# Francis-Fan-create/SCaSML_GP

Measured on AMD Instinct MI355X. Metric: Euler-Maruyama path-steps/sec + L2 rel-error, Grad_Dependent_Nonlinear d=100 n=3, higher is better.
Workload: dtype f32

## Files before the change

### scasml_gp_amd/csrc/gp_eval_compat_mfma.hip

```cpp
#include <stdlib.h>
#include <type_traits>

#include "gp_common.hpp"
#include "gp_mfma16.hpp"

namespace scasml {

constexpr int kHutch = 5;

typedef _Float16 h16x2 __attribute__((ext_vector_type(2)));
typedef float f32x2 __attribute__((ext_vector_type(2)));

struct CompatIdxF {
    int32_t i[kHutch];
};

struct GpCompatArgs {
    const float *points;
    const float *model;
    int32_t idx[kHutch];
    float4 *out4;
    float *lap;
    int64_t n_inf;
    int32_t n_pad, kp, d, first_bdy_tile;
    float a, sigma, mu;
    int32_t eq_id;
    int32_t round_out;
    const uint8_t *site_kinds;
    int64_t rows_per_site;
    const int32_t *site_order;
    int32_t n_listed;
};

template <bool R16>
struct Pair {
    using T = std::conditional_t<R16, h16x2, f32x2>;
    T v;
    __device__ __forceinline__ Pair(float a, float b) {
        if constexpr (R16) v = __builtin_convertvector((f32x2){a, b}, h16x2);
        else v = (f32x2){a, b};
    }
    __device__ __forceinline__ float lo() const { return (float)v.x; }
    __device__ __forceinline__ float hi() const { return (float)v.y; }
};

__device__ __forceinline__ float pin(float x) {
    asm("" : "+v"(x));
    return x;
}

template <int KS, int PLANES>
__device__ __forceinline__ void compat_mfma_lam(const float4 *lds_a, const s16x8 (&xb)[PLANES][KS], f32x16 &acc, int lane, float acc0) {
#pragma unroll
    for (int r = 0; r < 16; ++r) acc[r] = acc0;
    constexpr int NA = PLANES == 2 ? 1 : 2;
    Frag a[NA];
    if constexpr (NA == 2) a[0].f = lds_a[lane];
#pragma unroll
    for (int s = 0; s < KS; ++s) {
        const int cur = NA == 2 ? (s & 1) : 0, nxt = cur ^ 1;
        if constexpr (NA == 2) {
            if (s + 1 < KS) a[nxt].f = lds_a[(s + 1) * 64 + lane];
        } else {
            a[0].f = lds_a[s * 64 + lane];
        }
        Frag b0;
        b0.v = xb[0][s];
        if constexpr (PLANES == 2) {
            Frag b1;
            b1.v = xb[1][s];
            acc = __builtin_amdgcn_mfma_f32_32x32x16_f16(a[cur].h, b1.h, acc, 0, 0, 0);
        }
        acc = __builtin_amdgcn_mfma_f32_32x32x16_f16(a[cur].h, b0.h, acc, 0, 0, 0);
        __builtin_amdgcn_sched_barrier(0);
    }
}

struct CompatPoint {
    float sx, tx, ax0, sx2, wxa, wxb;
};
struct CompatConsts {
    float a, ad, c4, c10;
};

template <int GEOM, int FORM, bool BDY, bool R16>
__device__ __forceinline__ void compat_epilogue(const float *rows_lds, const f32x16 &lam, const f32x16 &G, int half, const CompatPoint &p,
                                                const CompatConsts &c, float &au, float &at, float &ad, float &al) {
    const float4 *cb = reinterpret_cast<const float4 *>(__builtin_assume_aligned(rows_lds + 4 * 8 * half, 16));
    constexpr int NQ = (BDY || GEOM == 1) ? 1 : 2;
    float4 q[1][NQ];
    auto fetch = [&](int r, float4 (&dst)[NQ]) {
        const int row = (r & 3) + 8 * (r >> 2);
#pragma unroll
        for (int i = 0; i < NQ; ++i) dst[i] = cb[row * 2 + i];
    };
#pragma unroll
    for (int r = 0; r < 16; ++r) {
        const int cur = 0;
        fetch(r, q[0]);
        __builtin_amdgcn_sched_barrier(0);
        const float kap = pin(__builtin_amdgcn_exp2f(lam[r]));
        if constexpr (GEOM == 0) {
            const float vsy = q[cur][0].x, vty = q[cur][0].y, c0 = q[cur][0].z;
            if constexpr (BDY && FORM == 1) {
                const Pair<R16> k0(kap, 0.0f);
                au = fmaf(c0, k0.lo(), au);
            } else {
                const float pp = p.tx - vty, ss = p.sx - vsy;
                const float e1 = pin(pp * kap), e2 = pin(ss * kap);
                if constexpr (BDY) {
                    const Pair<R16> k01(kap, e1), k2(e2, 0.0f);
                    au = fmaf(c0, k01.lo(), au);
                    if constexpr (FORM == 0) at = fmaf(-c0, k01.hi(), at);
                    if constexpr (FORM != 1) ad = fmaf(-c0, k2.lo(), ad);
                } else {
                    const float cL = q[cur][0].w, ct = q[cur][1].x, cS = q[cur][1].y;
                    if constexpr (FORM == 1) {
                        const Pair<R16> k01(kap, e1), k2(e2, 0.0f);
                        au = fmaf(cS, k2.lo(), fmaf(ct, k01.hi(), fmaf(c0, k01.lo(), au)));
                    } else {
                        const float e4 = pin(pp * e2);
                        const float e5 = pin(fmaf(-ss, e2, c.ad * kap));
                        if constexpr (FORM == 2) {
                            const Pair<R16> k01(kap, e1), k24(e2, e4), k5(e5, 0.0f);
                            au = fmaf(cS, k24.lo(), fmaf(ct, k01.hi(), fmaf(c0, k01.lo(), au)));
                            ad = fmaf(cS, k5.lo(), fmaf(-ct, k24.hi(), fmaf(-c0, k24.lo(), ad)));
                        } else {
                            const float e3 = fmaf(-pp, e1, c.a * kap);
                            const float g0 = G[r];
                            const float e6 = fmaf(g0, g0 - c.c4, -c.c10) * kap;
                            const Pair<R16> k01(kap, e1), k23(e2, e3), k45(e4, e5), k6(e6, 0.0f);
                            au = fmaf(cS, k23.lo(), fmaf(ct, k01.hi(), fmaf(c0, k01.lo(), au)));
                            at = fmaf(-cS, k45.lo(), fmaf(ct, k23.hi(), fmaf(-c0, k01.hi(), at)));
                            ad = fmaf(cS, k45.hi(), fmaf(-ct, k45.lo(), fmaf(-c0, k23.lo(), ad)));
                            al = fmaf(cL, k6.lo(), al);
                        }
                    }
                }
            }
        } else if constexpr (GEOM == 1) {
            const float vsy1 = q[cur][0].x, vay0 = q[cur][0].y, vwy1 = q[cur][0].z, cL = q[cur][0].w;
            const float g1 = G[r];
            const float f1 = pin(g1 * kap);
            if constexpr (FORM == 1) {
                const Pair<R16> k1(f1, 0.0f);
                au = fmaf(cL, k1.lo(), au);
            } else {
                const float m = fmaf(-(p.sx - vsy1), g1, p.wxb - vwy1);
                const float f3 = pin(m * kap);
                if constexpr (FORM == 2) {
                    const Pair<R16> k13(f1, f3);
                    au = fmaf(cL, k13.lo(), au);
                    ad = fmaf(cL, k13.hi(), ad);
                } else {
                    const float f2 = (p.tx - vay0) * f1;
                    const Pair<R16> k12(f1, f2), k3(f3, 0.0f);
                    au = fmaf(cL, k12.lo(), au);
                    at = fmaf(-cL, k12.hi(), at);
                    ad = fmaf(cL, k3.lo(), ad);
                }
            }
        } else {
            const float vsy = q[cur][0].x, vty = q[cur][0].y, vwy2 = q[cur][0].z, c0 = q[cur][0].w;
            const float g2 = G[r];
            const float h1 = g2 * kap;
            if constexpr (BDY) {
                const Pair<R16> k1(h1, 0.0f);
                al = fmaf(c0, k1.lo(), al);
            } else {
                const float ct = q[cur][1].x, cS = q[cur][1].y;
                const float h2 = (p.ax0 - vty) * h1;
                const float m = fmaf(-(p.sx2 - vsy), g2, p.wxa - vwy2);
                const float h3 = m * kap;
                const Pair<R16> k12(h1, h2), k3(h3, 0.0f);
                al = fmaf(-cS, k3.lo(), fmaf(ct, k12.hi(), fmaf(c0, k12.lo(), al)));
            }
        }
    }
}

template <int GEOM, int FORM, bool BDY>
__device__ __forceinline__ void compat_epilogue_fact(const float *rows_lds, const f32x16 &lam, const f32x16 &G, int half, const CompatPoint &p,
                                                     const CompatConsts &c, float &au, float &at, float &ad, float &al) {
    const float4 *cb = reinterpret_cast<const float4 *>(__builtin_assume_aligned(rows_lds + 4 * 8 * half, 16));
    constexpr int Q0 = GEOM == 2 ? 1 : 0;
    constexpr int NQ = (GEOM == 0 && !BDY) ? 2 : 1;
    float4 q[2][NQ];
    auto fetch = [&](int r, float4 (&dst)[NQ]) {
        const int row = (r & 3) + 8 * (r >> 2);
#pragma unroll
        for (int i = 0; i < NQ; ++i) dst[i] = cb[row * 2 + Q0 + i];
    };
    fetch(0, q[0]);
#pragma unroll
    for (int r = 0; r < 16; ++r) {
        const int cur = r & 1, nxt = cur ^ 1;
        if (r + 1 < 16) fetch(r + 1, q[nxt]);
        #ifndef SCASML_FACT_NOSCHED
        __builtin_amdgcn_sched_barrier(0);
#endif
        const float kap = __builtin_amdgcn_exp2f(lam[r]);
        if constexpr (GEOM == 0) {
            const float vsy = q[cur][0].x, vty = q[cur][0].y, c0 = q[cur][0].z;
            if constexpr (BDY) {
                const float F = c0 * kap;
                au += F;
                if constexpr (FORM == 0) at = fmaf(-(p.tx - vty), F, at);
                if constexpr (FORM != 1) ad = fmaf(-(p.sx - vsy), F, ad);
            } else {
                const float cL = q[cur][0].w, ct = q[cur][1].x, cS = q[cur][1].y;
                const float pp = p.tx - vty, ss = p.sx - vsy;
                const float E = fmaf(ct, pp, fmaf(cS, ss, c0));
                au = fmaf(kap, E, au);
                if constexpr (FORM != 1) ad = fmaf(kap, fmaf(-ss, E, q[cur][1].w), ad);
                if constexpr (FORM == 0) {
                    at = fmaf(kap, fmaf(-pp, E, q[cur][1].z), at);
                    const float g0 = G[r];
                    al = fmaf(cL * kap, fmaf(g0, g0 - c.c4, -c.c10), al);
                }
            }
        } else if constexpr (GEOM == 1) {
            const float vsy1 = q[cur][0].x, vay0 = q[cur][0].y, vwy1 = q[cur][0].z, cL = q[cur][0].w;
            const float v = cL * kap;
            if constexpr (FORM == 1) {
                au = fmaf(v, G[r], au);
            } else {
                const float w = v * G[r];
                au += w;
                ad = fmaf(-(p.sx - vsy1), w, fmaf(v, p.wxb - vwy1, ad));
                if constexpr (FORM == 0) at = fmaf(-(p.tx - vay0), w, at);
            }
        } else {
            const float ct = q[cur][0].x, cS = q[cur][0].y, e0 = q[cur][0].z, cSw = q[cur][0].w;
            if constexpr (BDY) {
                al = fmaf(kap * G[r], e0, al);
            } else {
                const float E2 = fmaf(ct, p.ax0, fmaf(cS, p.sx2, e0));
                const float t = fmaf(cS, p.wxa, -cSw);
                al = fmaf(kap, fmaf(G[r], E2, -t), al);
            }
        }
    }
}

constexpr int kStageTail = 256 + 256;

template <int KS, int BPC, bool R16, int PLANES>
__global__ __launch_bounds__(256, BPC) void gp_eval_compat_mfma_kernel(const GpCompatArgs g) {
    static_assert(PLANES == 2 || !R16, "the as-coded form keeps both point planes");
#ifndef SCASML_COMPAT_NSLOT
#define SCASML_COMPAT_NSLOT 3
#endif
    constexpr int WPB = 4, NSLOT = SCASML_COMPAT_NSLOT, AHEAD = 2;
    constexpr int STAGE = KS * 256 + kStageTail;
    constexpr int NCHUNK = STAGE / 256;
    constexpr int CLO = NCHUNK / WPB, CREM = NCHUNK % WPB;
    extern __shared__ __attribute__((aligned(16))) float lds[];
    const int lane = threadIdx.x & 63, wv = threadIdx.x >> 6;
    const int col = lane & 31, half = lane >> 5;
    const int64_t blk = blockIdx.x;
    int64_t p0 = (blk * WPB + wv) * 32;
    const int n_tiles = g.n_pad / 32;
    const int nb0 = g.first_bdy_tile < n_tiles ? g.first_bdy_tile : n_tiles;

    int form_listed = -1;
    if (g.site_order) {
        const int64_t wps = g.rows_per_site >> 5;
        bool all_u = true, all_ud = true;
        for (int w = 0; w < WPB; ++w) {
            const int64_t vs = (blk * WPB + w) / wps;
            if (vs >= g.n_listed) continue;
            const int k = g.site_kinds ? g.site_kinds[g.site_order[vs]] : 0;
            if (!(k == 1 || k == 3)) all_u = false;
            if (!(k == 1 || k == 3 || k == 4)) all_ud = false;
        }
        form_listed = all_u ? 1 : (all_ud ? 2 : 0);
        const int64_t vw = blk * WPB + wv, vs = vw / wps;
        p0 = vs < g.n_listed ? (int64_t)g.site_order[vs] * g.rows_per_site + (vw - vs * wps) * 32 : g.n_inf;
    }

    if (!g.site_order && g.site_kinds && g.rows_per_site >= 32) {
        const int64_t b0 = blk * WPB * 32;
        if (b0 < g.n_inf) {
            const int64_t b1 = (b0 + WPB * 32 < g.n_inf ? b0 + WPB * 32 : g.n_inf) - 1;
            bool unowned = true;
            for (int64_t s = b0 / g.rows_per_site; s <= b1 / g.rows_per_site; ++s)
                if (g.site_kinds[s] != 2) unowned = false;
            if (unowned) return;
        }
    }
    int form = 0;
    if (g.site_order) {
        form = form_listed;
    } else if (g.site_kinds && g.rows_per_site >= 32) {
        const int64_t b0 = blk * WPB * 32;
        const int64_t b1 = (b0 + WPB * 32 < g.n_inf ? b0 + WPB * 32 : g.n_inf) - 1;
        if (b0 < g.n_inf) {
            bool all_u = true, all_ud = true;
            for (int64_t s = b0 / g.rows_per_site; s <= b1 / g.rows_per_site; ++s) {
                const int k = g.site_kinds[s];
                if (k == 2) continue;
                if (!(k == 1 || k == 3)) all_u = false;
                if (!(k == 1 || k == 3 || k == 4)) all_ud = false;
            }
            form = all_u ? 1 : (all_ud ? 2 : 0);
        }
    }
    form = __builtin_amdgcn_readfirstlane(form);
    const int GD = form == 0 ? 3 : 2, GB = form == 0 ? 2 : 1;
    const int n_stages = nb0 * GD + (n_tiles - nb0) * GB;

    const int wvs = __builtin_amdgcn_readfirstlane(wv);
    const bool extra = wvs < CREM;
    const uint32_t lds_base = __builtin_amdgcn_readfirstlane((uint32_t)(uintptr_t)lds);
    auto stage_src = [&](int s) -> const float * {
        int tile, geom;
        if (s < nb0 * GD) {
            tile = s / GD;
            geom = s - tile * GD;
        } else {
            const int t = s - nb0 * GD;
            tile = nb0 + t / GB;
            geom = form == 0 ? 2 * (t - (t / GB) * GB) : 0;
        }
        return g.model + ((int64_t)tile * 3 + geom) * STAGE;
    };
    auto stage = [&](int s) {
        const uint32_t dst = lds_base + (uint32_t)((s % NSLOT) * STAGE) * 4u;
        const float *src = stage_src(s);
        auto chunk = [&](int c) { glds16_asm(src + c * 256, (uint32_t)lane * 16u, dst + (uint32_t)c * 1024u); };
#pragma unroll
        for (int i = 0; i < CLO; ++i) chunk(wvs + i * WPB);
        if (CREM && extra) chunk(wvs + CLO * WPB);
    };
    auto rendezvous = [&](bool newest_may_fly) {
        if (newest_may_fly) {
            if (CREM && extra) {
                asm volatile("s_waitcnt vmcnt(%0)" ::"n"(CLO + 1) : "memory");
            } else {
                asm volatile("s_waitcnt vmcnt(%0)" ::"n"(CLO) : "memory");
            }
        } else {
            asm volatile("s_waitcnt vmcnt(0)" ::: "memory");
        }
        __builtin_amdgcn_s_barrier();
        asm volatile("" ::: "memory");
    };
    stage(0);
    if (n_stages > 1) stage(1);

    const float qs = 0.5f * 1.44269504088896341f / g.a, k1 = -qs;
    const float hh = (float)g.d / (float)kHutch;
    const float ha2 = hh * g.a * g.a;
    s16x8 xb[PLANES][KS];
    float acc0 = 0.0f;
    CompatPoint pt;
    Frag qa[1], qb[1];
    {
        int64_t row = p0 + col;
        if (row >= g.n_inf) row = g.n_inf - 1;
        const float *prow = g.points + row * g.kp;
        const int kbase = half * (8 * KS);
        const float4 *src = reinterpret_cast<const float4 *>(prow + kbase);
        float pn = 0.0f, ps = 0.0f;
        const float ptime = prow[g.d], px0 = prow[0];
        const float fold = 2.0f * g.a * g.a * qs;
        auto make_planes = [&](const float (&t)[8], Frag &fh, Frag &fl) {
#pragma unroll
            for (int c = 0; c < 4; ++c) {
                const float h0 = (float)(_Float16)t[2 * c], h1 = (float)(_Float16)t[2 * c + 1];
                fh.u[c] = pack_h2(t[2 * c], t[2 * c + 1]);
                fl.u[c] = pack_h2(t[2 * c] - h0, t[2 * c + 1] - h1);
            }
        };
        float tlast[8];
#pragma unroll
        for (int s = 0; s < KS; ++s) {
            const float4 q0 = src[2 * s], q1 = src[2 * s + 1];
            const float e[8] = {q0.x, q0.y, q0.z, q0.w, q1.x, q1.y, q1.z, q1.w};
            float t[8];
#pragma unroll
            for (int c2 = 0; c2 < 8; ++c2) {
                pn = fmaf(e[c2], e[c2], pn);
                ps += e[c2];
                t[c2] = fold * e[c2];
            }
            if (s == KS - 1) {
#pragma unroll
                for (int c2 = 0; c2 < 8; ++c2) tlast[c2] = t[c2];
            } else {
                Frag fh, fl;
                make_planes(t, fh, fl);
                xb[0][s] = fh.v;
                if constexpr (PLANES == 2) xb[1][s] = fl.v;
            }
        }
        pn += __shfl_xor(pn, 32);
        ps += __shfl_xor(ps, 32);
        tlast[5] = half ? 1.0f : tlast[5];
        tlast[6] = half ? 1.0f : tlast[6];
        tlast[7] = half ? k1 * g.a * g.a * pn : tlast[7];
        {
            Frag fh, fl;
            make_planes(tlast, fh, fl);
            xb[0][KS - 1] = fh.v;
            if constexpr (PLANES == 2) xb[1][KS - 1] = fl.v;
            else acc0 = k1 * g.a * g.a * pn - (float)(_Float16)(k1 * g.a * g.a * pn);
        }
        pt.sx = g.a * (ps - ptime);
        pt.tx = g.a * ptime;
        pt.ax0 = g.a * px0;
        pt.sx2 = pt.sx - pt.ax0 + pt.tx;
        float ua[kHutch], ub[kHutch], sa = 0.0f, sb = 0.0f, na = 0.0f, nb = 0.0f;
#pragma unroll
        for (int j = 0; j < kHutch; ++j) {
            const float va = prow[g.idx[j] + 1], vb = prow[g.idx[j]];
            sa += va;
            sb += vb;
            na = fmaf(va, va, na);
            nb = fmaf(vb, vb, nb);
            ua[j] = -2.0f * ha2 * va;
            ub[j] = -2.0f * ha2 * vb;
        }
        pt.wxa = 2.0f * ha2 * sa;
        pt.wxb = 2.0f * ha2 * sb;
        auto qfrag = [&](const float (&u)[kHutch], float px, Frag &f) {
            auto hi = [](float v) { return (float)(_Float16)v; };
            if (half == 0) {
                f.u[0] = pack_h2(u[0], u[1]);
                f.u[1] = pack_h2(u[2], u[3]);
                f.u[2] = pack_h2(u[4], px);
                f.u[3] = pack_h2(px - hi(px), 1.0f);
            } else {
                f.u[0] = pack_h2(u[0] - hi(u[0]), u[1] - hi(u[1]));
                f.u[1] = pack_h2(u[2] - hi(u[2]), u[3] - hi(u[3]));
                f.u[2] = pack_h2(u[4] - hi(u[4]), 1.0f);
                f.u[3] = 0u;
            }
        };
        const float c5ah = (float)kHutch * g.a * hh;
        qfrag(ua, fmaf(ha2, na, -c5ah), qa[0]);
        qfrag(ub, fmaf(ha2, nb, -c5ah), qb[0]);
    }
    CompatConsts cc;
    cc.a = g.a;
    cc.ad = g.a * (float)g.d;
    cc.c4 = 4.0f * g.a * hh;
    cc.c10 = 10.0f * g.a * g.a * hh * hh;
    float au = 0.0f, at = 0.0f, ad = 0.0f, al = 0.0f;
    f32x16 acc, accG;
    uint32_t region;
    asm volatile("s_mov_b32 %0, -1" : "=s"(region));

    int s_now = 0;
    auto step = [&](auto geom_c, auto form_c, auto bdy_c) {
        constexpr int GEOM = decltype(geom_c)::value, FORM = decltype(form_c)::value;
        constexpr bool BDY = decltype(bdy_c)::value;
        constexpr bool NEEDG = GEOM != 0 || (FORM == 0 && !BDY);
        const int slot = s_now % NSLOT;
        if (s_now + AHEAD < n_stages) stage(s_now + AHEAD);
        const float *base = lds + slot * STAGE;
        if (region & 1) {
            compat_mfma_lam<KS, PLANES>(reinterpret_cast<const float4 *>(base), xb, acc, lane, acc0);
            if constexpr (NEEDG) {
                Frag aq;
                aq.f = reinterpret_cast<const float4 *>(base + KS * 256)[lane];
#pragma unroll
                for (int r = 0; r < 16; ++r) accG[r] = 0.0f;
                accG = __builtin_amdgcn_mfma_f32_32x32x16_f16(aq.h, GEOM == 1 ? qb[0].h : qa[0].h, accG, 0, 0, 0);
            }
        }
        if (region & 2) {
            if constexpr (R16) compat_epilogue<GEOM, FORM, BDY, true>(base + (KS + 1) * 256, acc, accG, half, pt, cc, au, at, ad, al);
            else compat_epilogue_fact<GEOM, FORM, BDY>(base + (KS + 1) * 256, acc, accG, half, pt, cc, au, at, ad, al);
        }
        rendezvous(s_now + AHEAD < n_stages);
        ++s_now;
    };
    using I0 = std::integral_constant<int, 0>;
    using I1 = std::integral_constant<int, 1>;
    using I2 = std::integral_constant<int, 2>;
    auto sweep = [&](auto form_c) {
        constexpr int FORM = decltype(form_c)::value;
        for (int jt = 0; jt < nb0; ++jt) {
            step(I0{}, form_c, std::false_type{});
            step(I1{}, form_c, std::false_type{});
            if constexpr (FORM == 0) step(I2{}, form_c, std::false_type{});
        }
        for (int jt = nb0; jt < n_tiles; ++jt) {
            step(I0{}, form_c, std::true_type{});
            if constexpr (FORM == 0) step(I2{}, form_c, std::true_type{});
        }
    };
    rendezvous(n_stages > 1);
    if (form == 2) sweep(I2{});
    else if (form == 1) sweep(I1{});
    else sweep(I0{});

    float u = au + __shfl_xor(au, 32);
    const float dt = at + __shfl_xor(at, 32);
    const float dv = ad + __shfl_xor(ad, 32);
    const float lp = al + __shfl_xor(al, 32);
    const int64_t row = p0 + col;
    if (half == 0 && row < g.n_inf) {
        if (g.round_out) u = (float)(_Float16)u;
        float eps = dt + g.mu * dv + 0.5f * g.sigma * g.sigma * lp + eq_f<float>(g.eq_id, u, g.sigma * dv, g.sigma, (float)g.d);
        if (g.round_out) eps = (float)(_Float16)eps;
        g.out4[row] = make_float4(u, dv, eps, dt);
        if (g.lap) g.lap[row] = lp;
    }
}

__global__ void gp_compat_pack_mfma_kernel(int d, float a, const float *x_dom, int n_dom, const float *x_bdy, int n_bdy, const double *rv,
                                           CompatIdxF ix, float *model, int n_pad, int kp) {
    const int j = blockIdx.x * blockDim.x + threadIdx.x;
    if (j >= n_pad) return;
    const int N = n_dom + n_bdy, D = d + 1, KS = kp / 16;
    const float *src = j < n_dom ? x_dom + (int64_t)j * D : (j < N ? x_bdy + (int64_t)(j - n_dom) * D : nullptr);
    auto y = [&](int k) { return src ? src[k] : 0.0f; };
    const float qs = 0.5f * 1.44269504088896341f / a, k1 = -qs;
    const float hh = (float)d / (float)kHutch, ha2 = hh * a * a;
    float ny = 0.0f, sy = 0.0f;
    for (int k = 0; k < D; ++k) ny = fmaf(y(k), y(k), ny);
    for (int k = 0; k < d; ++k) sy += y(k);
    const float ay = k1 * a * a * ny;
    const _Float16 ayh = (_Float16)ay;
    const float ayl = ay - (float)ayh;
    float c0 = 0.0f, cL = 0.0f, ct = 0.0f, cS = 0.0f;
    if (j < n_dom) {
        c0 = (float)rv[j];
        cL = (float)rv[N + j];
        ct = (float)rv[N + n_dom + j];
        cS = (float)rv[N + 2 * n_dom + j];
    } else if (j < N) {
        c0 = (float)rv[j];
    }
    const int tile = j / 32, i = j % 32;
    const int stage_floats = KS * 256 + kStageTail;
    for (int g = 0; g < 3; ++g) {
        float *blk = model + ((int64_t)tile * 3 + g) * stage_floats;
        uint16_t *planes = reinterpret_cast<uint16_t *>(blk);
        auto yg = [&](int k) { return g == 0 ? y(k) : (g == 1 ? y((k + 1) % D) : y((k + D - 1) % D)); };
        for (int k = 0; k < kp; ++k) {
            const float v = k <= d ? yg(k) : (k == kp - 3 ? (float)ayh : (k == kp - 2 ? ayl : (k == kp - 1 ? 1.0f : 0.0f)));
            const int h = k / (kp / 2), kk = k % (kp / 2);
            const int64_t e = (((int64_t)(kk / 8)) * 64 + h * 32 + i) * 8 + (kk & 7);
            planes[e] = __builtin_bit_cast(unsigned short, (_Float16)v);
        }
        float yq[kHutch], nq = 0.0f, sq = 0.0f;
        for (int q = 0; q < kHutch; ++q) {
            yq[q] = y(ix.i[q] + (g == 2 ? 0 : 1));
            nq = fmaf(yq[q], yq[q], nq);
            sq += yq[q];
        }
        const float py = ha2 * nq;
        const _Float16 pyh = (_Float16)py;
        uint16_t *qf = reinterpret_cast<uint16_t *>(blk + KS * 256);
        auto put = [&](int h, int e, float v) { qf[(h * 32 + i) * 8 + e] = __builtin_bit_cast(unsigned short, (_Float16)v); };
        for (int q = 0; q < kHutch; ++q) {
            put(0, q, yq[q]);
            put(1, q, yq[q]);
        }
        put(0, 5, 1.0f);
        put(0, 6, 1.0f);
        put(0, 7, (float)pyh);
        put(1, 5, py - (float)pyh);
        put(1, 6, 0.0f);
        put(1, 7, 0.0f);
        float *rc = blk + (KS + 1) * 256 + i * 8;
        for (int q = 0; q < 8; ++q) rc[q] = 0.0f;
        if (g == 0) {
            rc[0] = a * sy;
            rc[1] = a * y(d);
            rc[2] = c0;
            rc[3] = cL;
            rc[4] = ct;
            rc[5] = cS;
            rc[6] = a * ct;
            rc[7] = a * (float)d * cS;
        } else if (g == 1) {
            rc[0] = a * (sy - y(0) + y(d));
            rc[1] = a * y(0);
            rc[2] = 2.0f * ha2 * sq;
            rc[3] = cL;
        } else {
            rc[0] = a * sy;
            rc[1] = a * y(d);
            rc[2] = 2.0f * ha2 * sq;
            rc[3] = c0;
            rc[4] = ct;
            rc[5] = cS;
            rc[6] = fmaf(-cS, rc[0], fmaf(-ct, rc[1], c0));
            rc[7] = cS * rc[2];
        }
    }
}

template <int KS, bool R16, int PLANES>
static int launch_compat(const GpCompatArgs &g, hipStream_t s) {
    constexpr int REGS = 4 * PLANES * KS + (R16 ? 72 : 90);
    constexpr size_t lds_bytes = SCASML_COMPAT_NSLOT * (size_t)(KS * 256 + kStageTail) * sizeof(float);
    constexpr int BPC_REGS = REGS <= 128 ? 4 : (REGS <= 164 ? 3 : 2), BPC_LDS = (int)(160 * 1024 / lds_bytes);
    constexpr int BPC = BPC_REGS < BPC_LDS ? BPC_REGS : BPC_LDS;
    const int64_t waves = g.site_order ? (int64_t)g.n_listed * (g.rows_per_site >> 5) : (g.n_inf + 31) / 32;
    const int64_t blocks = (waves + 3) / 4;
    if (blocks == 0) return 0;
    if (blocks > 0x7FFFFFFF) return fail(SCASML_ERR_UNSUPPORTED, "gp_eval_compat_sites: too many points");
    static_assert(lds_bytes * BPC <= 160 * 1024, "LDS slots exceed 160 KiB");
    auto kern = gp_eval_compat_mfma_kernel<KS, BPC, R16, PLANES>;
    if (lds_bytes > 64 * 1024) {
        if (hipFuncSetAttribute(reinterpret_cast<const void *>(kern), hipFuncAttributeMaxDynamicSharedMemorySize, (int)lds_bytes) != hipSuccess)
            return fail(SCASML_ERR_HIP, "gp_eval_compat_sites: cannot reserve %zu bytes of LDS", lds_bytes);
    }
    hipLaunchKernelGGL(kern, dim3((unsigned)blocks), dim3(256), lds_bytes, s, g);
    return check_launch("gp_eval_compat_sites launch");
}

template <bool R16, int PLANES>
static int launch_compat_ks(const GpCompatArgs &g, hipStream_t s) {
    switch (g.kp / 16) {
#define SCASML_CASE(K) \
    case K: return launch_compat<K, R16, PLANES>(g, s);
        SCASML_CASE(1) SCASML_CASE(2) SCASML_CASE(3) SCASML_CASE(4) SCASML_CASE(5) SCASML_CASE(6) SCASML_CASE(7) SCASML_CASE(8)
        SCASML_CASE(9) SCASML_CASE(10) SCASML_CASE(11) SCASML_CASE(12) SCASML_CASE(13) SCASML_CASE(14) SCASML_CASE(15) SCASML_CASE(16)
#undef SCASML_CASE
    }
    return fail(SCASML_ERR_UNSUPPORTED, "gp_eval_compat_sites: kp=%d", g.kp);
}

static int check_idx5(const int32_t *idx_h, int d, int32_t (&out)[kHutch], const char *who) {
    if (!idx_h) return fail(SCASML_ERR_ARG, "%s: idx is null", who);
    for (int j = 0; j < kHutch; ++j) {
        if (idx_h[j] < 0 || idx_h[j] >= d) return fail(SCASML_ERR_ARG, "%s: idx[%d] = %d outside [0, d)", who, j, idx_h[j]);
        for (int q = 0; q < j; ++q)
            if (idx_h[q] == idx_h[j]) return fail(SCASML_ERR_ARG, "%s: idx has a repeated entry %d", who, idx_h[j]);
        out[j] = idx_h[j];
    }
    return 0;
}

}

using namespace scasml;

extern "C" int64_t scasml_gp_compat_model_floats(int32_t d, int32_t n_pad) {
    const int64_t kp = scasml_point_stride(d);
    return (int64_t)(n_pad / SCASML_GP_TILE) * 3 * ((kp / 16) * 256 + kStageTail);
}

extern "C" int scasml_gp_compat_pack_mfma(int32_t d, float a, const float *x_dom, int32_t n_dom, const float *x_bdy, int32_t n_bdy,
                                          const double *rv, const int32_t *idx_h, float *model_out, void *stream) {
    if (!x_dom || !rv || !model_out || (n_bdy > 0 && !x_bdy)) return fail(SCASML_ERR_ARG, "gp_compat_pack_mfma: null argument");
    if (d < kHutch || d > SCASML_MAX_DIM || n_dom < 1 || n_bdy < 0) return fail(SCASML_ERR_ARG, "gp_compat_pack_mfma: bad sizes (d >= %d needed)", kHutch);
    CompatIdxF ix;
    if (int rc = check_idx5(idx_h, d, ix.i, "gp_compat_pack_mfma")) return rc;
    const int n_pad = (n_dom + n_bdy + 31) / 32 * 32;
    const int kp = scasml_point_stride(d);
    hipLaunchKernelGGL(gp_compat_pack_mfma_kernel, dim3((n_pad + 63) / 64), dim3(64), 0, (hipStream_t)stream, d, a, x_dom, n_dom, x_bdy, n_bdy,
                       rv, ix, model_out, n_pad, kp);
    return check_launch("gp_compat_pack_mfma launch");
}

static int eval_compat_sites(int32_t d, float a, float sigma_eq, float mu_eq, int32_t eq_id, const float *model, int32_t n_dom,
                             int32_t n_bdy, const int32_t *idx_h, int32_t round16, float x_bound, const float *points, int64_t n_inf,
                             int64_t rows_per_site, const uint8_t *site_kinds, const int32_t *site_order, int32_t n_listed, float *out4, float *lap,
                             void *stream);

extern "C" int scasml_gp_eval_compat_sites(int32_t d, float a, float sigma_eq, float mu_eq, int32_t eq_id, const float *model, int32_t n_dom,
                                           int32_t n_bdy, const int32_t *idx_h, int32_t round16, float x_bound, const float *points, int64_t n_inf,
                                           int64_t rows_per_site, const uint8_t *site_kinds, float *out4, float *lap, void *stream) {
    return eval_compat_sites(d, a, sigma_eq, mu_eq, eq_id, model, n_dom, n_bdy, idx_h, round16, x_bound, points, n_inf, rows_per_site, site_kinds, nullptr,
                             0, out4, lap, stream);
}

extern "C" int scasml_gp_eval_compat_site_list(int32_t d, float a, float sigma_eq, float mu_eq, int32_t eq_id, const float *model, int32_t n_dom,
                                               int32_t n_bdy, const int32_t *idx_h, int32_t round16, float x_bound, const float *points, int64_t n_inf,
                                               int64_t rows_per_site, const uint8_t *site_kinds, const int32_t *site_order, int32_t n_listed,
                                               float *out4, float *lap, void *stream) {
    if (!site_order || n_listed < 0) return fail(SCASML_ERR_ARG, "gp_eval_compat_site_list: null or negative site list");
    if (rows_per_site < 32 || (rows_per_site & 31)) return fail(SCASML_ERR_ARG, "gp_eval_compat_site_list: rows_per_site must be a positive multiple of 32");
    if (n_inf % rows_per_site) return fail(SCASML_ERR_ARG, "gp_eval_compat_site_list: n_inf must be a whole number of sites");
    if (n_listed > n_inf / rows_per_site) return fail(SCASML_ERR_ARG, "gp_eval_compat_site_list: %d listed sites, the buffer holds %lld", n_listed, (long long)(n_inf / rows_per_site));
    if (n_listed == 0) return 0;
    return eval_compat_sites(d, a, sigma_eq, mu_eq, eq_id, model, n_dom, n_bdy, idx_h, round16, x_bound, points, n_inf, rows_per_site, site_kinds, site_order,
                             n_listed, out4, lap, stream);
}

static int eval_compat_sites(int32_t d, float a, float sigma_eq, float mu_eq, int32_t eq_id, const float *model, int32_t n_dom,
                             int32_t n_bdy, const int32_t *idx_h, int32_t round16, float x_bound, const float *points, int64_t n_inf,
                             int64_t rows_per_site, const uint8_t *site_kinds, const int32_t *site_order, int32_t n_listed, float *out4, float *lap,
                             void *stream) {
    if (n_inf == 0) return 0;
    if (!model || !points || !out4 || n_inf < 0) return fail(SCASML_ERR_ARG, "gp_eval_compat_sites: bad argument");
    if (d < kHutch || d > SCASML_MAX_DIM || n_dom < 1 || n_bdy < 0) return fail(SCASML_ERR_ARG, "gp_eval_compat_sites: bad sizes");
    if (site_kinds && rows_per_site < 1) return fail(SCASML_ERR_ARG, "gp_eval_compat_sites: rows_per_site must be positive");
    if (!eq_known(eq_id)) return fail(SCASML_ERR_UNSUPPORTED, "gp_eval_compat_sites: unknown equation id %d", eq_id);
    const float xb = x_bound > 0.0f ? x_bound : 2.0f;
    if (0.7213f * a * xb * xb * (float)(d + 1) > 3.0e4f)
        return fail(SCASML_ERR_UNSUPPORTED, "gp_eval_compat_sites: a = %g with |x_k| <= %g is outside the fp16 range at d = %d; use scasml_gp_eval_compat",
                    (double)a, (double)xb, d);
    GpCompatArgs g;
    if (int rc = check_idx5(idx_h, d, g.idx, "gp_eval_compat_sites")) return rc;
    g.points = points;
    g.model = model;
    g.out4 = reinterpret_cast<float4 *>(out4);
    g.lap = lap;
    g.n_inf = n_inf;
    g.n_pad = (n_dom + n_bdy + 31) / 32 * 32;
    g.kp = scasml_point_stride(d);
    g.d = d;
    g.first_bdy_tile = (n_dom + SCASML_GP_TILE - 1) / SCASML_GP_TILE;
    g.a = a;
    g.sigma = sigma_eq;
    g.mu = mu_eq;
    g.eq_id = eq_id;
    g.round_out = (round16 & 2) ? 1 : 0;
    g.site_kinds = site_kinds;
    g.rows_per_site = rows_per_site;
    g.site_order = site_order;
    g.n_listed = n_listed;
    hipStream_t s = (hipStream_t)stream;
    if (round16 & 1) {
        if (round16 & 4) return fail(SCASML_ERR_ARG, "gp_eval_compat_sites: round16 bit 2 (one point plane) is the geometry mode's option, not the as-coded form's");
        return launch_compat_ks<true, 2>(g, s);
    }
    return (round16 & 4) ? launch_compat_ks<false, 1>(g, s) : launch_compat_ks<false, 2>(g, s);
}
```

Measured before the change: 501.8 million.

## Pack hi/lo planes of the sparse tail k-slice into one MFMA operand

When the last 16-wide k-slice holds few real coordinates (d+1 leaves room), the model packing now places the high and low fp16 planes of that tail slice in the two halves of a single fragment, so the two-plane kernel issues one MFMA instead of two for the final step. The column layout of the packed model and the in-kernel point fragments are reorganised to match, and a separate tail kernel instantiation is selected at launch. It also makes the row base wave-uniform via readfirstlane. This adds layout complexity and new template variants, and correctness depends on the packer and evaluator agreeing on the tail map.

```diff
diff --git a/scasml_gp_amd/csrc/gp_eval_compat_mfma.hip b/scasml_gp_amd/csrc/gp_eval_compat_mfma.hip
--- a/scasml_gp_amd/csrc/gp_eval_compat_mfma.hip
+++ b/scasml_gp_amd/csrc/gp_eval_compat_mfma.hip
@@ -30,6 +30,7 @@
     int64_t rows_per_site;
     const int32_t *site_order;
     int32_t n_listed;
+    int32_t tail_packed;
 };
 
 template <bool R16>
@@ -49,7 +50,12 @@
     return x;
 }
 
-template <int KS, int PLANES>
+static inline bool compat_tail_packed(int d, int kp) {
+    const int r = d + 1 - (kp - 16);
+    return 2 * (r > 0 ? r : 0) + 4 <= 16;
+}
+
+template <int KS, int PLANES, bool PACK>
 __device__ __forceinline__ void compat_mfma_lam(const float4 *lds_a, const s16x8 (&xb)[PLANES][KS], f32x16 &acc, int lane, float acc0) {
 #pragma unroll
     for (int r = 0; r < 16; ++r) acc[r] = acc0;
@@ -67,9 +73,11 @@
         Frag b0;
         b0.v = xb[0][s];
         if constexpr (PLANES == 2) {
-            Frag b1;
-            b1.v = xb[1][s];
-            acc = __builtin_amdgcn_mfma_f32_32x32x16_f16(a[cur].h, b1.h, acc, 0, 0, 0);
+            if (!(PACK && s == KS - 1)) {
+                Frag b1;
+                b1.v = xb[1][s];
+                acc = __builtin_amdgcn_mfma_f32_32x32x16_f16(a[cur].h, b1.h, acc, 0, 0, 0);
+            }
         }
         acc = __builtin_amdgcn_mfma_f32_32x32x16_f16(a[cur].h, b0.h, acc, 0, 0, 0);
         __builtin_amdgcn_sched_barrier(0);
@@ -245,8 +253,8 @@
 
 constexpr int kStageTail = 256 + 256;
 
-template <int KS, int BPC, bool R16, int PLANES>
-__global__ __launch_bounds__(256, BPC) void gp_eval_compat_mfma_kernel(const GpCompatArgs g) {
+template <int KS, bool R16, int PLANES, bool PACK>
+__device__ __forceinline__ void compat_mfma_sweep(const GpCompatArgs g) {
     static_assert(PLANES == 2 || !R16, "the as-coded form keeps both point planes");
 #ifndef SCASML_COMPAT_NSLOT
 #define SCASML_COMPAT_NSLOT 3
@@ -279,6 +287,8 @@
         p0 = vs < g.n_listed ? (int64_t)g.site_order[vs] * g.rows_per_site + (vw - vs * wps) * 32 : g.n_inf;
     }
 
+    p0 = ((int64_t)__builtin_amdgcn_readfirstlane((int32_t)(p0 >> 32)) << 32) | (uint32_t)__builtin_amdgcn_readfirstlane((int32_t)p0);
+
     if (!g.site_order && g.site_kinds && g.rows_per_site >= 32) {
         const int64_t b0 = blk * WPB * 32;
         if (b0 < g.n_inf) {
@@ -360,32 +370,34 @@
         int64_t row = p0 + col;
         if (row >= g.n_inf) row = g.n_inf - 1;
         const float *prow = g.points + row * g.kp;
-        const int kbase = half * (8 * KS);
-        const float4 *src = reinterpret_cast<const float4 *>(prow + kbase);
+        const float4 *src = reinterpret_cast<const float4 *>(prow + half * (8 * (KS - 1)));
+        const float4 *src_tail = reinterpret_cast<const float4 *>(prow + 16 * (KS - 1) + (PACK ? 0 : 8 * half));
         float pn = 0.0f, ps = 0.0f;
         const float ptime = prow[g.d], px0 = prow[0];
         const float fold = 2.0f * g.a * g.a * qs;
+        auto lo = [](float v) { return v - (float)(_Float16)v; };
         auto make_planes = [&](const float (&t)[8], Frag &fh, Frag &fl) {
 #pragma unroll
             for (int c = 0; c < 4; ++c) {
-                const float h0 = (float)(_Float16)t[2 * c], h1 = (float)(_Float16)t[2 * c + 1];
                 fh.u[c] = pack_h2(t[2 * c], t[2 * c + 1]);
-                fl.u[c] = pack_h2(t[2 * c] - h0, t[2 * c + 1] - h1);
+                fl.u[c] = pack_h2(lo(t[2 * c]), lo(t[2 * c + 1]));
             }
         };
         float tlast[8];
 #pragma unroll
         for (int s = 0; s < KS; ++s) {
-            const float4 q0 = src[2 * s], q1 = src[2 * s + 1];
+            const bool last = s == KS - 1;
+            const float4 q0 = last ? src_tail[0] : src[2 * s], q1 = last ? src_tail[1] : src[2 * s + 1];
             const float e[8] = {q0.x, q0.y, q0.z, q0.w, q1.x, q1.y, q1.z, q1.w};
             float t[8];
 #pragma unroll
             for (int c2 = 0; c2 < 8; ++c2) {
-                pn = fmaf(e[c2], e[c2], pn);
-                ps += e[c2];
+                const float w = (PACK && last && half) ? 0.0f : e[c2];
+                pn = fmaf(w, w, pn);
+                ps += w;
                 t[c2] = fold * e[c2];
             }
-            if (s == KS - 1) {
+            if (last) {
 #pragma unroll
                 for (int c2 = 0; c2 < 8; ++c2) tlast[c2] = t[c2];
             } else {
@@ -397,15 +409,34 @@
         }
         pn += __shfl_xor(pn, 32);
         ps += __shfl_xor(ps, 32);
-        tlast[5] = half ? 1.0f : tlast[5];
-        tlast[6] = half ? 1.0f : tlast[6];
-        tlast[7] = half ? k1 * g.a * g.a * pn : tlast[7];
-        {
+        const float x2 = k1 * g.a * g.a * pn;
+        if constexpr (PLANES == 1) {
+            const bool packed = g.tail_packed != 0;
+            tlast[5] = half ? (packed ? 0.0f : 1.0f) : tlast[5];
+            tlast[6] = half ? (packed ? x2 : 1.0f) : (packed ? 1.0f : tlast[6]);
+            tlast[7] = half ? (packed ? 0.0f : x2) : (packed ? 1.0f : tlast[7]);
             Frag fh, fl;
             make_planes(tlast, fh, fl);
             xb[0][KS - 1] = fh.v;
-            if constexpr (PLANES == 2) xb[1][KS - 1] = fl.v;
-            else acc0 = k1 * g.a * g.a * pn - (float)(_Float16)(k1 * g.a * g.a * pn);
+            acc0 = lo(x2);
+        } else if constexpr (PACK) {
+            Frag f;
+#pragma unroll
+            for (int c = 0; c < 3; ++c) {
+                const uint32_t h2 = pack_h2(tlast[2 * c], tlast[2 * c + 1]);
+                const uint32_t l2 = pack_h2(lo(tlast[2 * c]), lo(tlast[2 * c + 1]));
+                f.u[c] = half ? l2 : h2;
+            }
+            f.u[3] = half ? pack_h2(x2, lo(x2)) : pack_h2(1.0f, 1.0f);
+            xb[0][KS - 1] = f.v;
+        } else {
+            tlast[5] = half ? 1.0f : tlast[5];
+            tlast[6] = half ? 1.0f : tlast[6];
+            tlast[7] = half ? x2 : tlast[7];
+            Frag fh, fl;
+            make_planes(tlast, fh, fl);
+            xb[0][KS - 1] = fh.v;
+            xb[1][KS - 1] = fl.v;
         }
         pt.sx = g.a * (ps - ptime);
         pt.tx = g.a * ptime;
@@ -461,7 +492,7 @@
         if (s_now + AHEAD < n_stages) stage(s_now + AHEAD);
         const float *base = lds + slot * STAGE;
         if (region & 1) {
-            compat_mfma_lam<KS, PLANES>(reinterpret_cast<const float4 *>(base), xb, acc, lane, acc0);
+            compat_mfma_lam<KS, PLANES, PACK>(reinterpret_cast<const float4 *>(base), xb, acc, lane, acc0);
             if constexpr (NEEDG) {
                 Frag aq;
                 aq.f = reinterpret_cast<const float4 *>(base + KS * 256)[lane];
@@ -501,7 +532,9 @@
     const float dt = at + __shfl_xor(at, 32);
     const float dv = ad + __shfl_xor(ad, 32);
     const float lp = al + __shfl_xor(al, 32);
-    const int64_t row = p0 + col;
+    int col_out = col;
+    if constexpr (R16) asm volatile("" : "+v"(col_out));
+    const int64_t row = p0 + col_out;
     if (half == 0 && row < g.n_inf) {
         if (g.round_out) u = (float)(_Float16)u;
         float eps = dt + g.mu * dv + 0.5f * g.sigma * g.sigma * lp + eq_f<float>(g.eq_id, u, g.sigma * dv, g.sigma, (float)g.d);
@@ -511,8 +544,18 @@
     }
 }
 
+template <int KS, int BPC, bool R16, int PLANES>
+__global__ __launch_bounds__(256, BPC) void gp_eval_compat_mfma_kernel(const GpCompatArgs g) {
+    compat_mfma_sweep<KS, R16, PLANES, false>(g);
+}
+
+template <int KS, int BPC, bool R16, int PLANES>
+__global__ __launch_bounds__(256, BPC) void gp_eval_compat_mfma_tail_kernel(const GpCompatArgs g) {
+    compat_mfma_sweep<KS, R16, PLANES, true>(g);
+}
+
 __global__ void gp_compat_pack_mfma_kernel(int d, float a, const float *x_dom, int n_dom, const float *x_bdy, int n_bdy, const double *rv,
-                                           CompatIdxF ix, float *model, int n_pad, int kp) {
+                                           CompatIdxF ix, float *model, int n_pad, int kp, int packed) {
     const int j = blockIdx.x * blockDim.x + threadIdx.x;
     if (j >= n_pad) return;
     const int N = n_dom + n_bdy, D = d + 1, KS = kp / 16;
@@ -541,11 +584,17 @@
         float *blk = model + ((int64_t)tile * 3 + g) * stage_floats;
         uint16_t *planes = reinterpret_cast<uint16_t *>(blk);
         auto yg = [&](int k) { return g == 0 ? y(k) : (g == 1 ? y((k + 1) % D) : y((k + D - 1) % D)); };
-        for (int k = 0; k < kp; ++k) {
-            const float v = k <= d ? yg(k) : (k == kp - 3 ? (float)ayh : (k == kp - 2 ? ayl : (k == kp - 1 ? 1.0f : 0.0f)));
-            const int h = k / (kp / 2), kk = k % (kp / 2);
-            const int64_t e = (((int64_t)(kk / 8)) * 64 + h * 32 + i) * 8 + (kk & 7);
-            planes[e] = __builtin_bit_cast(unsigned short, (_Float16)v);
+        for (int s = 0; s < KS; ++s) {
+            for (int c = 0; c < 16; ++c) {
+                const int k = s < KS - 1 ? (c >> 3) * 8 * (KS - 1) + 8 * s + (c & 7)
+                                         : 16 * s + (packed && c >= 8 ? c - 8 : c);
+                float v = k <= d ? yg(k) : 0.0f;
+                if (s == KS - 1) {
+                    if (packed) v = (c & 7) < 6 ? v : (c == 6 ? (float)ayh : (c == 7 ? ayl : 1.0f));
+                    else v = c < 13 ? v : (c == 13 ? (float)ayh : (c == 14 ? ayl : 1.0f));
+                }
+                planes[(((int64_t)s * 64 + (c >> 3) * 32 + i) * 8) + (c & 7)] = __builtin_bit_cast(unsigned short, (_Float16)v);
+            }
         }
         float yq[kHutch], nq = 0.0f, sq = 0.0f;
         for (int q = 0; q < kHutch; ++q) {
@@ -596,7 +645,7 @@
     }
 }
 
-template <int KS, bool R16, int PLANES>
+template <int KS, bool R16, int PLANES, bool PACK>
 static int launch_compat(const GpCompatArgs &g, hipStream_t s) {
     constexpr int REGS = 4 * PLANES * KS + (R16 ? 72 : 90);
     constexpr size_t lds_bytes = SCASML_COMPAT_NSLOT * (size_t)(KS * 256 + kStageTail) * sizeof(float);
@@ -607,7 +656,9 @@
     if (blocks == 0) return 0;
     if (blocks > 0x7FFFFFFF) return fail(SCASML_ERR_UNSUPPORTED, "gp_eval_compat_sites: too many points");
     static_assert(lds_bytes * BPC <= 160 * 1024, "LDS slots exceed 160 KiB");
-    auto kern = gp_eval_compat_mfma_kernel<KS, BPC, R16, PLANES>;
+    void (*kern)(const GpCompatArgs) = gp_eval_compat_mfma_kernel<KS, BPC, R16, PLANES>;
+    if constexpr (PACK) kern = gp_eval_compat_mfma_tail_kernel<KS, BPC, R16, PLANES>;
+    static_assert(PLANES == 2 || !PACK, "one plane: one kernel for both column maps");
     if (lds_bytes > 64 * 1024) {
         if (hipFuncSetAttribute(reinterpret_cast<const void *>(kern), hipFuncAttributeMaxDynamicSharedMemorySize, (int)lds_bytes) != hipSuccess)
             return fail(SCASML_ERR_HIP, "gp_eval_compat_sites: cannot reserve %zu bytes of LDS", lds_bytes);
@@ -618,9 +669,14 @@
 
 template <bool R16, int PLANES>
 static int launch_compat_ks(const GpCompatArgs &g, hipStream_t s) {
+    const bool packed = PLANES == 2 && g.tail_packed;
     switch (g.kp / 16) {
 #define SCASML_CASE(K) \
-    case K: return launch_compat<K, R16, PLANES>(g, s);
+    case K:                                                                                \
+        if constexpr (PLANES == 2) {                                                       \
+            if (packed) return launch_compat<K, R16, PLANES, true>(g, s);                   \
+        }                                                                                  \
+        return launch_compat<K, R16, PLANES, false>(g, s);
         SCASML_CASE(1) SCASML_CASE(2) SCASML_CASE(3) SCASML_CASE(4) SCASML_CASE(5) SCASML_CASE(6) SCASML_CASE(7) SCASML_CASE(8)
         SCASML_CASE(9) SCASML_CASE(10) SCASML_CASE(11) SCASML_CASE(12) SCASML_CASE(13) SCASML_CASE(14) SCASML_CASE(15) SCASML_CASE(16)
 #undef SCASML_CASE
@@ -657,7 +713,7 @@
     const int n_pad = (n_dom + n_bdy + 31) / 32 * 32;
     const int kp = scasml_point_stride(d);
     hipLaunchKernelGGL(gp_compat_pack_mfma_kernel, dim3((n_pad + 63) / 64), dim3(64), 0, (hipStream_t)stream, d, a, x_dom, n_dom, x_bdy, n_bdy,
-                       rv, ix, model_out, n_pad, kp);
+                       rv, ix, model_out, n_pad, kp, compat_tail_packed(d, kp) ? 1 : 0);
     return check_launch("gp_compat_pack_mfma launch");
 }
 
@@ -719,6 +775,7 @@
     g.rows_per_site = rows_per_site;
     g.site_order = site_order;
     g.n_listed = n_listed;
+    g.tail_packed = compat_tail_packed(d, g.kp) ? 1 : 0;
     hipStream_t s = (hipStream_t)stream;
     if (round16 & 1) {
         if (round16 & 4) return fail(SCASML_ERR_ARG, "gp_eval_compat_sites: round16 bit 2 (one point plane) is the geometry mode's option, not the as-coded form's");
```

New measurement: 510.2 million (median of 6 runs). +1.7%, better.
